# VachaLab/gorder

Measured on AMD Instinct MI355X. Metric: trajectory frames/sec, higher is better.
Workload: dtype f32

## Files before the change

### gorder_amd/csrc/trajectory_driver.h

```cpp
#pragma once

#include <atomic>
#include <chrono>
#include <condition_variable>
#include <deque>
#include <mutex>
#include <thread>

#include "../../include/gorder_xtc.h"

namespace {

struct TrajSlot {
    float *h_xyz = nullptr, *h_box = nullptr, *h_time = nullptr;
    float *d_xyz = nullptr, *d_box = nullptr;
    uint8_t *h_blob = nullptr, *d_blob = nullptr;
    gorder_xtc_frame_t *h_frames = nullptr, *d_frames = nullptr;
    float *d_box_in = nullptr;
    uint32_t *d_stat = nullptr, *d_short = nullptr, *h_stat = nullptr, *h_short = nullptr;
    XtcCheckpoint *d_cp = nullptr;
    std::vector<int64_t> file_pos;
    std::vector<uint32_t> file_idx;
    uint32_t prefix_q16 = 65536;
    uint32_t kinds = 0;
// ... 279 lines not shown
            {
                std::lock_guard<std::mutex> lk(pipe.mu);
                if (pipe.stop) return;
            }
            const auto t0 = std::chrono::steady_clock::now();
            const hipError_t e = alloc_slot(pipe.slot[k]);
            std::lock_guard<std::mutex> lk(pipe.mu);
            pipe.setup_s += seconds_since(t0);
            if (e != hipSuccess) { pipe.alloc_failed = true; return; }
            pipe.free_q.push_back(k);
            pipe.cv.notify_all();
        }
    });
    const double setup_s = seconds_since(t_start);

    gorder_xtc_pool *pool = nullptr;
    if (dev && gorder_xtc_pool_create(n_threads, &pool) != GORDER_XTC_OK) pool = nullptr;
    const char *forced_prefix = getenv("GORDER_HIP_PREFIX_Q16");
    const bool adapt_prefix = dev && has_xtc && !forced_prefix && !env_flag("GORDER_HIP_NO_PREFIX") && n_stop < n_file_atoms;
    if (dev && forced_prefix) pipe.prefix_q16.store((uint32_t)std::max(1l, std::min(65536l, atol(forced_prefix))));
    const bool verify = dev && has_xtc && (adapt_prefix || forced_prefix);
    const int device = h->device;
    std::thread reader([&, device]() {
        (void)hipSetDevice(device);
        uint64_t state = 0, analysed = shard_lo;
        double last_time = -INFINITY;
        uint32_t f = 0;
        gorder_xtc_reader *r = nullptr;
        bool done = shard_n == 0;
        uint32_t n_filled = 0;
        uint64_t to_skip = shard_lo, left = shard_n;
        auto give_up = [&](int st, const std::string &msg) {
            std::lock_guard<std::mutex> lk(pipe.mu);
            pipe.reader_status = st;
            pipe.reader_msg = msg;
            done = true;
        };
        while (!done) {
            int k = -1;
            {
                const auto t0 = std::chrono::steady_clock::now();
                std::unique_lock<std::mutex> lk(pipe.mu);
                pipe.cv.wait(lk, [&] { return pipe.stop || !pipe.free_q.empty(); });
                pipe.reader_stalled_s += seconds_since(t0);
                if (pipe.stop) break;
                k = pipe.free_q.front();
                pipe.free_q.pop_front();
            }
            TrajSlot &s = pipe.slot[k];
            const auto t_wait = std::chrono::steady_clock::now();
            if (s.copy_issued) (void)hipEventSynchronize(s.staged);
            const auto t1 = std::chrono::steady_clock::now();
            {
                std::lock_guard<std::mutex> lk(pipe.mu);
                pipe.reader_stalled_s += std::chrono::duration<double>(t1 - t_wait).count();
            }
            s.n = 0;
            s.blob_bytes = 0;
            uint32_t fill = batch;
            if (adapt_prefix && tr->batch_frames == 0 && f < tr->n_paths && file_is_xtc[f]) {
                if (n_filled == 0) fill = std::min(batch, 256u);
                else if (n_filled == 1) fill = std::min(batch, 1024u);
                else if (n_filled == 2) {
                    std::unique_lock<std::mutex> lk(pipe.mu);
                    pipe.cv.wait(lk, [&] { return pipe.stop || pipe.reports > 0; });
                }
            }
            s.prefix_q16 = pipe.prefix_q16.load();
            while (!done && s.n < fill) {
                if (left == 0) { done = true; break; }
                if (!r) {
                    if (f == tr->n_paths) { done = true; break; }
                    int st = gorder_xtc_open(tr->paths[f], tr->group, tr->n_group, &r);
                    if (st == GORDER_XTC_OK && gorder_xtc_n_atoms_out(r) != n_atoms) st = GORDER_XTC_ERR_ARGUMENT;
                    if (st != GORDER_XTC_OK) {
                        give_up(st, std::string("cannot read ") + tr->paths[f] +
                                        (st == GORDER_XTC_ERR_ARGUMENT ? ": atoms per frame differ from the tables" : ""));
                        break;
                    }
                }
                if (to_skip) {
                    const int64_t sk = gorder_xtc_skip_window(r, tr->begin_ps, tr->end_ps, tr->step, &state, &last_time, to_skip);
                    if (sk < 0) { give_up((int)sk, std::string("read error in ") + tr->paths[f]); break; }
                    to_skip -= (uint64_t)sk;
                    if (to_skip) {
                        gorder_xtc_close(r);
                        r = nullptr;
                        f++;
                        continue;
                    }
                }
                const uint64_t want = std::min<uint64_t>(fill - s.n, left);
                uint64_t used = 0;
                const int64_t got =
                    dev ? gorder_xtc_pack_window_ex(r, tr->begin_ps, tr->end_ps, tr->step, &state, &last_time,
                                                    s.h_blob + s.blob_bytes, blob_cap - s.blob_bytes, &used, s.h_frames + s.n,
                                                    s.h_box + 9u * (size_t)s.n, s.h_time + s.n, want, n_threads, pool,
                                                    s.prefix_q16, s.file_pos.data() + s.n)
                        : gorder_xtc_read_window_mt(r, tr->begin_ps, tr->end_ps, tr->step, &state, &last_time,
                                                    s.h_xyz + (size_t)s.n * n_atoms * 3u, s.h_box + 9u * (size_t)s.n,
                                                    s.h_time + s.n, want, n_threads);
                if (dev && got == GORDER_XTC_ERR_NO_SPACE) {
                    if (s.n > 0) break;
                    give_up(GORDER_XTC_ERR_ARGUMENT, std::string("a single frame of ") + tr->paths[f] + " does not fit the staging blob");
                    break;
                }
                if (got < 0) {
                    give_up((int)got, std::string("read error in ") + tr->paths[f]);
                    break;
                }
                if (got == 0) {
                    gorder_xtc_close(r);
                    r = nullptr;
                    f++;
                    continue;
                }
                if (dev) {
                    for (int64_t q = 0; q < got; q++) {
                        s.h_frames[s.n + (size_t)q].offset += s.blob_bytes;
                        s.file_idx[s.n + (size_t)q] = f;
                    }
                    s.blob_bytes += used;
                }
                s.n += (uint32_t)got;
                left -= (uint64_t)got;
            }
            if (pool) {
                const int cst = gorder_xtc_pool_wait(pool);
                if (cst != GORDER_XTC_OK && !done) give_up(cst, "read error while copying the compressed blocks");
                else if (cst != GORDER_XTC_OK) { std::lock_guard<std::mutex> lk(pipe.mu); if (pipe.reader_status == GORDER_XTC_OK) { pipe.reader_status = cst; pipe.reader_msg = "read error while copying the compressed blocks"; } }
            }
            const double dt = seconds_since(t1);
            std::lock_guard<std::mutex> lk(pipe.mu);
            pipe.decode_s += dt;
            if (s.n == 0 || pipe.reader_status != GORDER_XTC_OK) {
                pipe.free_q.push_front(k);
                break;
            }
            if (dev && (xtc_table_kinds(s.h_frames, s.n) & kXtcTableXtc)) n_filled++;
            s.fidx.resize((size_t)s.n);
            for (uint32_t q = 0; q < s.n; q++) s.fidx[q] = tr->first_frame_index + (analysed + q) * tr->step;
            analysed += s.n;
            pipe.filled_q.push_back(k);
            pipe.cv.notify_all();
        }
        if (r) gorder_xtc_close(r);
        std::lock_guard<std::mutex> lk(pipe.mu);
        pipe.reader_done = true;
        pipe.cv.notify_all();
    });

    int status = GORDER_OK;
    uint64_t frames = 0, batches = 0, bytes = 0, frames_fixed = 0;
    double starved_s = 0.0;
    std::string hip_msg;
    uint32_t need_q16 = 0;
    auto stage_a = [&](int k) {
        TrajSlot &s = pipe.slot[k];
        const size_t nx = (size_t)s.n * n_atoms * 3u * sizeof(float), nb = (size_t)s.n * 9u * sizeof(float);
        hipError_t e = hipSuccess;
        const hipStream_t feed = dev ? s.stream : copy_stream;
        if (s.compute_issued && !dev) e = hipStreamWaitEvent(feed, s.computed, 0);
// ... 124 lines not shown
            go = stage_b(front);
            any = true;
        }
        if (go && !any && !decoding.empty()) {
            std::unique_lock<std::mutex> lk(pipe.mu);
            pipe.cv.wait_for(lk, std::chrono::microseconds(100), [&] { return !pipe.filled_q.empty(); });
        }
    }
    {
        std::lock_guard<std::mutex> lk(pipe.mu);
        pipe.stop = true;
        pipe.cv.notify_all();
    }
    reader.join();
    allocator.join();
    if (pool) gorder_xtc_pool_destroy(pool);
    (void)hipStreamSynchronize(copy_stream);
    for (int k = 0; k < TrajPipe::kSlots; k++)
        if (pipe.slot[k].stream) (void)hipStreamSynchronize(pipe.slot[k].stream);
    const int sync_status = gorder_hip_synchronize(h);
    if (status == GORDER_OK) status = sync_status;
    else if (!hip_msg.empty()) h->err_msg = hip_msg;
    if (status == GORDER_OK && pipe.reader_status != GORDER_XTC_OK) {
        status = pipe.reader_status == GORDER_XTC_ERR_FORMAT ? GORDER_ERR_TRAJECTORY_FORMAT : GORDER_ERR_INVALID_ARGUMENT;
        h->err_msg = pipe.reader_msg + " (reader status " + std::to_string(pipe.reader_status) + ")";
    }
    if (stats) {
        stats->n_frames = frames;
        stats->n_batches = batches;
        stats->bytes_h2d = bytes;
        stats->seconds_total = seconds_since(t_start);
// ... 17 lines not shown
```

### gorder_amd/csrc/xtc_reader.cpp

```cpp
#include <algorithm>
#include <climits>
#include <cmath>
#include <cstdint>
#include <cstdio>
#include <cstring>
#include <string>
#include <string>
#include <atomic>
#include <chrono>
#include <condition_variable>
#include <deque>
#include <functional>
#include <memory>
#include <mutex>
#include <thread>
#include <immintrin.h>
#include <sys/mman.h>
#include <sys/stat.h>
#include <unistd.h>
#include <vector>

#include "../../include/gorder_xtc.h"

namespace {

const int kMagicInts[] = {
    0,       0,       0,       0,       0,       0,       0,       0,       0,       8,        10,       12,
    16,      20,      25,      32,      40,      50,      64,      80,      101,     128,      161,      203,
    256,     322,     406,     512,     645,     812,     1024,    1290,    1625,    2048,     2580,     3250,
    4096,    5060,    6501,    8192,    10321,   13003,   16384,   20642,   26007,   32768,    41285,    52015,
    65536,   82570,   104031,  131072,  165140,  208063,  262144,  330280,  416127,  524287,   660561,   832255,
    1048576, 1321122, 1664510, 2097152, 2642245, 3329021, 4194304, 5284491, 6658042, 8388607,  10568983, 13316085,
// ... 119 lines not shown
    float f;
    memcpy(&f, &u, 4);
    return f;
}

double bed(const uint8_t *p) {
    uint64_t u = 0;
    for (int k = 0; k < 8; k++) u = (u << 8) | p[k];
    double d;
    memcpy(&d, &u, 8);
    return d;
}

}

struct FileMap {
    const uint8_t *base = nullptr;
    size_t size = 0;
    ~FileMap() { if (base) munmap(const_cast<uint8_t *>(base), size); }
};

struct gorder_xtc_reader {
    std::string path;
    FILE *fp = nullptr;
    bool trr = false;
    bool gro = false;
    uint32_t natoms = 0;
    std::vector<uint32_t> group;
    std::vector<int32_t> slot_of;
    uint32_t n_needed = 0;
    std::vector<uint8_t> buf;
    std::vector<int> ints;
    std::shared_ptr<struct FileMap> map;
    bool map_tried = false;
};

namespace {

bool read_exact(FILE *fp, void *dst, size_t n) { return fread(dst, 1, n, fp) == n; }

int decode_ints(gorder_xtc_reader *r, const int minint[3], const int maxint[3], int smallidx, const uint8_t *data,
                size_t nbytes) {
    const uint32_t natoms = r->natoms;
    r->ints.resize((size_t)natoms * 3);
    uint32_t sizeint[3];
    int bitsizeint[3] = {0, 0, 0};
    for (int k = 0; k < 3; k++) {
        const int64_t s = (int64_t)maxint[k] - (int64_t)minint[k] + 1;
        if (s <= 0 || s > 0xffffffffll) return GORDER_XTC_ERR_FORMAT;
// ... 654 lines not shown
                float t = 0.0f;
                st = gorder_xtc_next(mine, xyz + i * nout * 3, box9 + i * 9, nullptr, &t, nullptr);
                if (st == GORDER_XTC_OK && time_ps) time_ps[i] = t;
            }
            gorder_xtc_close(mine);
            status[w] = st;
        });
    for (auto &th : pool) th.join();
    for (int st : status)
        if (st != GORDER_XTC_OK) return st == GORDER_XTC_EOF ? GORDER_XTC_ERR_FORMAT : st;
    return (int64_t)n;
}

}

struct gorder_xtc_pool {
    std::vector<std::thread> workers;
    std::mutex mu;
    std::condition_variable cv_work, cv_idle;
    std::deque<std::function<int()>> jobs;
    size_t running = 0;
    int status = GORDER_XTC_OK;
    bool stop = false;
    void loop() {
        for (;;) {
            std::function<int()> job;
            {
                std::unique_lock<std::mutex> lk(mu);
                cv_work.wait(lk, [&] { return stop || !jobs.empty(); });
                if (jobs.empty()) return;
                job = std::move(jobs.front());
                jobs.pop_front();
                running++;
            }
            const int st = job();
            std::lock_guard<std::mutex> lk(mu);
            if (st != GORDER_XTC_OK && status == GORDER_XTC_OK) status = st;
            running--;
            if (jobs.empty() && running == 0) cv_idle.notify_all();
        }
    }
};

extern "C" {

int gorder_xtc_pool_create(uint32_t n_threads, gorder_xtc_pool **out) {
    if (!out) return GORDER_XTC_ERR_ARGUMENT;
    gorder_xtc_pool *p = new gorder_xtc_pool();
    for (uint32_t w = 0; w < std::max(1u, n_threads); w++) p->workers.emplace_back([p] { p->loop(); });
    *out = p;
    return GORDER_XTC_OK;
}
int gorder_xtc_pool_wait(gorder_xtc_pool *p) {
    if (!p) return GORDER_XTC_ERR_ARGUMENT;
    std::unique_lock<std::mutex> lk(p->mu);
    p->cv_idle.wait(lk, [&] { return p->jobs.empty() && p->running == 0; });
    const int st = p->status;
    p->status = GORDER_XTC_OK;
    return st;
}
void gorder_xtc_pool_destroy(gorder_xtc_pool *p) {
    if (!p) return;
    {
        std::lock_guard<std::mutex> lk(p->mu);
// ... 74 lines not shown
    for (; i + 128 <= n; i += 128) {
        const __m256i a = _mm256_loadu_si256((const __m256i *)(src + i)), b = _mm256_loadu_si256((const __m256i *)(src + i + 32));
        const __m256i c = _mm256_loadu_si256((const __m256i *)(src + i + 64)), d = _mm256_loadu_si256((const __m256i *)(src + i + 96));
        _mm256_stream_si256((__m256i *)(dst + i), a);
        _mm256_stream_si256((__m256i *)(dst + i + 32), b);
        _mm256_stream_si256((__m256i *)(dst + i + 64), c);
        _mm256_stream_si256((__m256i *)(dst + i + 96), d);
    }
    if (i < n) memcpy(dst + i, src + i, n - i);
    _mm_sfence();
}
bool have_avx2() {
    static const bool yes = __builtin_cpu_supports("avx2");
    return yes;
}
int pack_copy(int fd, const FileMap *map, const PackSrc *src, size_t i0, size_t i1, uint8_t *blob) {
    const bool stream = map && map->base && have_avx2() && !getenv("GORDER_XTC_PREAD");
    for (size_t i = i0; i < i1; i++) {
        uint8_t *dst = blob + src[i].dst;
        size_t done = 0;
        if (stream && ((uintptr_t)dst & 31u) == 0 && (size_t)src[i].pos + src[i].n <= map->size) {
            stream_copy_avx2(dst, map->base + src[i].pos, src[i].n);
            done = src[i].n;
        }
        while (done < src[i].n) {
            const ssize_t g = pread(fd, dst + done, src[i].n - done, src[i].pos + (off_t)done);
            if (g <= 0) return GORDER_XTC_ERR_FORMAT;
            done += (size_t)g;
        }
        const size_t end = (size_t)((((uint64_t)src[i].n + 63u) & ~63ull) + 64u);
        memset(dst + src[i].n, 0, end - src[i].n);
    }
    return GORDER_XTC_OK;
}

int64_t pack_window_impl(gorder_xtc_reader *r, float begin_ps, float end_ps, uint32_t step, uint64_t *state,
                         double *last_time, uint8_t *blob, uint64_t blob_capacity, uint64_t *blob_bytes,
                         gorder_xtc_frame_t *frames, float *box9, float *time_ps, uint64_t capacity,
                         uint32_t n_threads, gorder_xtc_pool *pool, uint32_t prefix_q16 = 65536u, int64_t *file_pos = nullptr) {
    if (!r || !r->fp || r->gro || !state || !last_time || !blob || !blob_bytes || !frames || !box9 || step == 0)
        return GORDER_XTC_ERR_ARGUMENT;
    *blob_bytes = 0;
    const auto t_scan0 = std::chrono::steady_clock::now();
    std::vector<PackSrc> src;
    uint64_t used = 0;
    const uint32_t natoms = r->natoms;
    const int fd = fileno(r->fp);
    off_t pos = (off_t)ftello(r->fp);
    bool to_end = false;
    const uint64_t state_at_entry = *state;
    const double last_time_at_entry = *last_time;
    struct stat sb;
    const off_t file_end = fstat(fd, &sb) == 0 && S_ISREG(sb.st_mode) ? sb.st_size : (off_t)-1;
    if (!r->map_tried) {
        r->map_tried = true;
        if (file_end > 0) {
            void *m = mmap(nullptr, (size_t)file_end, PROT_READ, MAP_SHARED, fd, 0);
            if (m != MAP_FAILED) {
                (void)madvise(m, (size_t)file_end, MADV_SEQUENTIAL);
                r->map = std::make_shared<FileMap>();
                r->map->base = static_cast<const uint8_t *>(m);
                r->map->size = (size_t)file_end;
            }
        }
    }
    if (r->map && (getenv("GORDER_XTC_PREAD") || (file_end >= 0 && (size_t)file_end < r->map->size))) r->map.reset();
    const FileMap *map = r->map.get();
    auto fetch = [&](off_t at, uint8_t *dst, size_t n) -> ssize_t {
        if (map && map->base && at >= 0 && (size_t)at + n <= map->size) {
            memcpy(dst, map->base + at, n);
            return (ssize_t)n;
        }
        return pread(fd, dst, n, at);
    };
    const uint32_t n_stop = gorder_xtc_n_atoms_needed(r);
    while (src.size() < capacity) {
        const off_t pos0 = pos;
        uint8_t head[56 + 36];
        float t;
        float trr_box[9] = {0.0f, 0.0f, 0.0f, 0.0f, 0.0f, 0.0f, 0.0f, 0.0f, 0.0f};
        gorder_xtc_frame_t fr{};
        uint32_t block = 0;
        uint32_t copy = 0;
        off_t pos_block;
// ... 86 lines not shown
        }
        const size_t i = src.size();
        fr.offset = used;
        used += need;
        frames[i] = fr;
        for (int q = 0; q < 9; q++) box9[9 * i + q] = r->trr ? trr_box[q] : bef(head + 16 + 4 * q);
        if (time_ps) time_ps[i] = t;
        if (file_pos) file_pos[i] = (int64_t)pos0;
        src.push_back({pos_block, copy, fr.offset});
    }
    if (to_end ? fseek(r->fp, 0, SEEK_END) != 0 : fseeko(r->fp, pos, SEEK_SET) != 0) return GORDER_XTC_ERR_FORMAT;
    const size_t n = src.size();
    if (n == 0) return 0;
    const auto t_copy0 = std::chrono::steady_clock::now();
    if (pool) {
        const size_t nj = std::min<size_t>(pool->workers.size(), n);
        auto shared = std::make_shared<std::vector<PackSrc>>(std::move(src));
        const int fd2 = dup(fd);
        if (fd2 < 0) return GORDER_XTC_ERR_OPEN;
        auto left = std::make_shared<std::atomic<size_t>>(nj);
        std::shared_ptr<FileMap> keep = r->map;
        {
            std::lock_guard<std::mutex> lk(pool->mu);
            for (size_t w = 0; w < nj; w++) {
                const size_t i0 = n * w / nj, i1 = n * (w + 1) / nj;
                pool->jobs.emplace_back([shared, fd2, left, i0, i1, blob, keep]() {
                    const int st = pack_copy(fd2, keep.get(), shared->data(), i0, i1, blob);
                    if (left->fetch_sub(1) == 1) close(fd2);
                    return st;
                });
            }
        }
        pool->cv_work.notify_all();
        *blob_bytes = used;
        return (int64_t)n;
    }
    const uint32_t nt = (uint32_t)std::min<size_t>(std::max(1u, n_threads), n);
    std::vector<int> status(nt, GORDER_XTC_OK);
    auto work = [&](uint32_t w) { status[w] = pack_copy(fd, map, src.data(), n * w / nt, n * (w + 1) / nt, blob); };
    if (nt == 1) {
        work(0);
    } else {
        std::vector<std::thread> threads;
        for (uint32_t w = 0; w < nt; w++) threads.emplace_back(work, w);
        for (auto &th : threads) th.join();
    }
    for (int st : status)
        if (st != GORDER_XTC_OK) return st;
    if (getenv("GORDER_XTC_PACK_TIMING")) {
        const auto t1 = std::chrono::steady_clock::now();
        fprintf(stderr, "pack_window: %zu frames, scan %.3f ms, copy %.3f ms (%u threads, %.1f MB)\n", n,
                std::chrono::duration<double, std::milli>(t_copy0 - t_scan0).count(),
                std::chrono::duration<double, std::milli>(t1 - t_copy0).count(), nt, used / 1e6);
    }
// ... 24 lines not shown
    if (!r || !r->fp || !xyz) return GORDER_XTC_ERR_ARGUMENT;
    if (fseeko(r->fp, (off_t)file_pos, SEEK_SET) != 0) return GORDER_XTC_ERR_FORMAT;
    return gorder_xtc_next(r, xyz, box9, nullptr, nullptr, nullptr);
}

int64_t gorder_xtc_pack_window_pool(gorder_xtc_reader *r, float begin_ps, float end_ps, uint32_t step, uint64_t *state,
                                    double *last_time, uint8_t *blob, uint64_t blob_capacity, uint64_t *blob_bytes,
                                    gorder_xtc_frame_t *frames, float *box9, float *time_ps, uint64_t capacity,
                                    gorder_xtc_pool *pool) {
    if (!pool) return GORDER_XTC_ERR_ARGUMENT;
    return pack_window_impl(r, begin_ps, end_ps, step, state, last_time, blob, blob_capacity, blob_bytes, frames, box9,
                            time_ps, capacity, 1, pool);
}

}
```

### gorder_amd/xtc.py

```python
from __future__ import annotations

import ctypes as C
from typing import Optional, Sequence

import numpy as np

from .abi import load_library

_bound = False


def _lib():
    global _bound
    lib = load_library()
    if not _bound:
        vp = C.c_void_p
        lib.gorder_xtc_open.argtypes = [C.c_char_p, vp, C.c_uint32, C.POINTER(vp)]
        lib.gorder_xtc_close.argtypes = [vp]
        lib.gorder_xtc_close.restype = None
        lib.gorder_xtc_n_atoms_file.argtypes = [vp]
        lib.gorder_xtc_n_atoms_file.restype = C.c_uint32
        lib.gorder_xtc_n_atoms_out.argtypes = [vp]
        lib.gorder_xtc_n_atoms_out.restype = C.c_uint32
        lib.gorder_xtc_next.argtypes = [vp, vp, vp, C.POINTER(C.c_int64), C.POINTER(C.c_float), C.POINTER(C.c_float)]
# ... 223 lines not shown
    state, last = C.c_uint64(0), C.c_double(float("-inf"))
    total = 0
    for path in paths:
        r = C.c_void_p()
        st = lib.gorder_xtc_open(path.encode(), None, 0, C.byref(r))
        if st != 0:
            raise IOError(f"cannot open {path}: status {st}")
        try:
            n = lib.gorder_xtc_skip_window(r, begin, end, step, C.byref(state), C.byref(last), 2 ** 64 - 1)
            if n < 0:
                raise IOError(f"{path}: XTC read error {n}")
            total += n
        finally:
            lib.gorder_xtc_close(r)
    return total
```

### include/gorder_xtc.h

```cpp
#ifndef GORDER_XTC_H
#define GORDER_XTC_H

#include <stddef.h>
#include <stdint.h>

#ifdef __cplusplus
extern "C" {
#endif

typedef struct gorder_xtc_reader gorder_xtc_reader;

typedef enum {
    GORDER_XTC_OK = 0,
    GORDER_XTC_EOF = 1,
    GORDER_XTC_ERR_OPEN = -1,
    GORDER_XTC_ERR_FORMAT = -2,
    GORDER_XTC_ERR_ARGUMENT = -3,
    GORDER_XTC_ERR_NO_SPACE = -4
} gorder_xtc_status_t;

int gorder_xtc_open(const char *path, const uint32_t *group, uint32_t n_group, gorder_xtc_reader **out);
void gorder_xtc_close(gorder_xtc_reader *r);
uint32_t gorder_xtc_n_atoms_file(const gorder_xtc_reader *r);
uint32_t gorder_xtc_n_atoms_out(const gorder_xtc_reader *r);
// ... 32 lines not shown
typedef struct gorder_xtc_pool gorder_xtc_pool;
int gorder_xtc_pool_create(uint32_t n_threads, gorder_xtc_pool **out);
int gorder_xtc_pool_wait(gorder_xtc_pool *pool);
void gorder_xtc_pool_destroy(gorder_xtc_pool *pool);
int64_t gorder_xtc_pack_window_pool(gorder_xtc_reader *r, float begin_ps, float end_ps, uint32_t step, uint64_t *state,
                                    double *last_time, uint8_t *blob, uint64_t blob_capacity, uint64_t *blob_bytes,
                                    gorder_xtc_frame_t *frames, float *box9, float *time_ps, uint64_t capacity,
                                    gorder_xtc_pool *pool);

int64_t gorder_xtc_pack_window_ex(gorder_xtc_reader *r, float begin_ps, float end_ps, uint32_t step, uint64_t *state,
                                  double *last_time, uint8_t *blob, uint64_t blob_capacity, uint64_t *blob_bytes,
                                  gorder_xtc_frame_t *frames, float *box9, float *time_ps, uint64_t capacity,
                                  uint32_t n_threads, gorder_xtc_pool *pool, uint32_t prefix_q16, int64_t *file_pos);
int gorder_xtc_read_at(gorder_xtc_reader *r, int64_t file_pos, float *xyz, float *box9);

int gorder_xtc_probe(const char *path, uint32_t *n_atoms, uint64_t *file_bytes, uint32_t *first_frame_bytes);
enum { GORDER_XTC_FORMAT_OTHER = 0, GORDER_XTC_FORMAT_XTC = 1, GORDER_XTC_FORMAT_TRR = 2 };
int gorder_xtc_probe_format(const char *path, int *format, uint32_t *n_atoms, uint64_t *file_bytes,
                            uint32_t *first_frame_bytes);
int gorder_xtc_is_xtc(const gorder_xtc_reader *r);
int gorder_xtc_can_pack(const gorder_xtc_reader *r);
uint32_t gorder_xtc_n_atoms_needed(const gorder_xtc_reader *r);

typedef struct gorder_xtc_writer gorder_xtc_writer;
int gorder_xtc_writer_open(const char *path, uint32_t n_atoms, float precision, gorder_xtc_writer **out);
int gorder_xtc_writer_add(gorder_xtc_writer *w, const float *xyz, const float *box9, int64_t step, float time_ps);
void gorder_xtc_writer_close(gorder_xtc_writer *w);

#ifdef __cplusplus
}
// ... 3 lines not shown
```

Measured before the change: 21.07 million.

## Add trajectory feeder with ticketed async block copies and background unmap reaper

Replaces the reader thread's inline open/skip/pack loop with a new feeder object. The feeder hands out tickets for the pooled compressed-block copies, so the reader can start filling the next slot before publishing the previous one, keeping one batch in flight. File unmapping (madvise DONTNEED plus munmap) moves to a background reaper thread, taking page-release cost off the critical path. Staging-event waits now run only when the event is still pending. This adds more threads and ordering complexity, which could cause races or extra contention.

Measured after the change: 20.40 million. 3.2% lower.

```diff
diff --git a/gorder_amd/csrc/trajectory_driver.h b/gorder_amd/csrc/trajectory_driver.h
--- a/gorder_amd/csrc/trajectory_driver.h
+++ b/gorder_amd/csrc/trajectory_driver.h
@@ -317,8 +317,7 @@
     });
     const double setup_s = seconds_since(t_start);
 
-    gorder_xtc_pool *pool = nullptr;
-    if (dev && gorder_xtc_pool_create(n_threads, &pool) != GORDER_XTC_OK) pool = nullptr;
+    const bool feed_timing = getenv("GORDER_XTC_PACK_TIMING") != nullptr;
     const char *forced_prefix = getenv("GORDER_HIP_PREFIX_Q16");
     const bool adapt_prefix = dev && has_xtc && !forced_prefix && !env_flag("GORDER_HIP_NO_PREFIX") && n_stop < n_file_atoms;
     if (dev && forced_prefix) pipe.prefix_q16.store((uint32_t)std::max(1l, std::min(65536l, atol(forced_prefix))));
@@ -326,129 +325,150 @@
     const int device = h->device;
     std::thread reader([&, device]() {
         (void)hipSetDevice(device);
-        uint64_t state = 0, analysed = shard_lo;
-        double last_time = -INFINITY;
-        uint32_t f = 0;
-        gorder_xtc_reader *r = nullptr;
+        const auto t_reader = std::chrono::steady_clock::now();
+        double stalled = 0.0;
+        uint64_t analysed = shard_lo;
         bool done = shard_n == 0;
         uint32_t n_filled = 0;
-        uint64_t to_skip = shard_lo, left = shard_n;
+        gorder_xtc_feed *feed = nullptr;
+        {
+            gorder_xtc_feed_config_t fc{};
+            fc.paths = tr->paths;
+            fc.n_paths = tr->n_paths;
+            fc.group = tr->group;
+            fc.n_group = tr->n_group;
+            fc.begin_ps = tr->begin_ps;
+            fc.end_ps = tr->end_ps;
+            fc.step = tr->step;
+            fc.n_atoms_out = n_atoms;
+            fc.skip_frames = shard_lo;
+            fc.max_frames = shard_n;
+            fc.n_threads = n_threads;
+            fc.flags = feed_timing ? GORDER_XTC_FEED_TIMING : 0u;
+            if (!done && gorder_xtc_feed_open(&fc, &feed) != GORDER_XTC_OK) feed = nullptr;
+        }
         auto give_up = [&](int st, const std::string &msg) {
             std::lock_guard<std::mutex> lk(pipe.mu);
-            pipe.reader_status = st;
-            pipe.reader_msg = msg;
+            if (pipe.reader_status == GORDER_XTC_OK) {
+                pipe.reader_status = st;
+                pipe.reader_msg = msg;
+            }
             done = true;
         };
+        if (!done && !feed) give_up(GORDER_XTC_ERR_ARGUMENT, "cannot start the trajectory feeder");
+        struct Pending { int k; uint64_t ticket; };
+        std::deque<Pending> pending;
+        bool copy_failed = false;
+        auto publish_oldest = [&]() {
+            const Pending p = pending.front();
+            pending.pop_front();
+            TrajSlot &s = pipe.slot[p.k];
+            const int cst = gorder_xtc_feed_wait(feed, p.ticket);
+            if (cst != GORDER_XTC_OK && !copy_failed) {
+                give_up(cst, "read error while copying the compressed blocks");
+                copy_failed = true;
+            }
+            std::lock_guard<std::mutex> lk(pipe.mu);
+            if (copy_failed) {
+                pipe.free_q.push_front(p.k);
+                return;
+            }
+            s.fidx.resize((size_t)s.n);
+            for (uint32_t q = 0; q < s.n; q++) s.fidx[q] = tr->first_frame_index + (analysed + q) * tr->step;
+            analysed += s.n;
+            pipe.filled_q.push_back(p.k);
+            pipe.cv.notify_all();
+        };
+        auto publish_all = [&]() { while (!pending.empty()) publish_oldest(); };
         while (!done) {
             int k = -1;
             {
+                std::unique_lock<std::mutex> lk(pipe.mu);
+                if (pipe.stop) break;
+                if (!pipe.free_q.empty()) {
+                    k = pipe.free_q.front();
+                    pipe.free_q.pop_front();
+                }
+            }
+            if (k < 0) {
+                publish_all();
                 const auto t0 = std::chrono::steady_clock::now();
                 std::unique_lock<std::mutex> lk(pipe.mu);
                 pipe.cv.wait(lk, [&] { return pipe.stop || !pipe.free_q.empty(); });
-                pipe.reader_stalled_s += seconds_since(t0);
+                stalled += seconds_since(t0);
                 if (pipe.stop) break;
                 k = pipe.free_q.front();
                 pipe.free_q.pop_front();
             }
             TrajSlot &s = pipe.slot[k];
-            const auto t_wait = std::chrono::steady_clock::now();
-            if (s.copy_issued) (void)hipEventSynchronize(s.staged);
-            const auto t1 = std::chrono::steady_clock::now();
-            {
-                std::lock_guard<std::mutex> lk(pipe.mu);
-                pipe.reader_stalled_s += std::chrono::duration<double>(t1 - t_wait).count();
+            if (s.copy_issued && hipEventQuery(s.staged) != hipSuccess) {
+                publish_all();
+                const auto t_wait = std::chrono::steady_clock::now();
+                (void)hipEventSynchronize(s.staged);
+                stalled += seconds_since(t_wait);
             }
             s.n = 0;
             s.blob_bytes = 0;
             uint32_t fill = batch;
+            const uint32_t f = gorder_xtc_feed_next_file(feed);
             if (adapt_prefix && tr->batch_frames == 0 && f < tr->n_paths && file_is_xtc[f]) {
                 if (n_filled == 0) fill = std::min(batch, 256u);
                 else if (n_filled == 1) fill = std::min(batch, 1024u);
                 else if (n_filled == 2) {
+                    publish_all();
                     std::unique_lock<std::mutex> lk(pipe.mu);
                     pipe.cv.wait(lk, [&] { return pipe.stop || pipe.reports > 0; });
                 }
             }
             s.prefix_q16 = pipe.prefix_q16.load();
-            while (!done && s.n < fill) {
-                if (left == 0) { done = true; break; }
-                if (!r) {
-                    if (f == tr->n_paths) { done = true; break; }
-                    int st = gorder_xtc_open(tr->paths[f], tr->group, tr->n_group, &r);
-                    if (st == GORDER_XTC_OK && gorder_xtc_n_atoms_out(r) != n_atoms) st = GORDER_XTC_ERR_ARGUMENT;
-                    if (st != GORDER_XTC_OK) {
-                        give_up(st, std::string("cannot read ") + tr->paths[f] +
-                                        (st == GORDER_XTC_ERR_ARGUMENT ? ": atoms per frame differ from the tables" : ""));
-                        break;
-                    }
-                }
-                if (to_skip) {
-                    const int64_t sk = gorder_xtc_skip_window(r, tr->begin_ps, tr->end_ps, tr->step, &state, &last_time, to_skip);
-                    if (sk < 0) { give_up((int)sk, std::string("read error in ") + tr->paths[f]); break; }
-                    to_skip -= (uint64_t)sk;
-                    if (to_skip) {
-                        gorder_xtc_close(r);
-                        r = nullptr;
-                        f++;
-                        continue;
-                    }
-                }
-                const uint64_t want = std::min<uint64_t>(fill - s.n, left);
-                uint64_t used = 0;
-                const int64_t got =
-                    dev ? gorder_xtc_pack_window_ex(r, tr->begin_ps, tr->end_ps, tr->step, &state, &last_time,
-                                                    s.h_blob + s.blob_bytes, blob_cap - s.blob_bytes, &used, s.h_frames + s.n,
-                                                    s.h_box + 9u * (size_t)s.n, s.h_time + s.n, want, n_threads, pool,
-                                                    s.prefix_q16, s.file_pos.data() + s.n)
-                        : gorder_xtc_read_window_mt(r, tr->begin_ps, tr->end_ps, tr->step, &state, &last_time,
-                                                    s.h_xyz + (size_t)s.n * n_atoms * 3u, s.h_box + 9u * (size_t)s.n,
-                                                    s.h_time + s.n, want, n_threads);
-                if (dev && got == GORDER_XTC_ERR_NO_SPACE) {
-                    if (s.n > 0) break;
-                    give_up(GORDER_XTC_ERR_ARGUMENT, std::string("a single frame of ") + tr->paths[f] + " does not fit the staging blob");
-                    break;
-                }
-                if (got < 0) {
-                    give_up((int)got, std::string("read error in ") + tr->paths[f]);
-                    break;
-                }
-                if (got == 0) {
-                    gorder_xtc_close(r);
-                    r = nullptr;
-                    f++;
-                    continue;
-                }
-                if (dev) {
-                    for (int64_t q = 0; q < got; q++) {
-                        s.h_frames[s.n + (size_t)q].offset += s.blob_bytes;
-                        s.file_idx[s.n + (size_t)q] = f;
-                    }
-                    s.blob_bytes += used;
-                }
-                s.n += (uint32_t)got;
-                left -= (uint64_t)got;
-            }
-            if (pool) {
-                const int cst = gorder_xtc_pool_wait(pool);
-                if (cst != GORDER_XTC_OK && !done) give_up(cst, "read error while copying the compressed blocks");
-                else if (cst != GORDER_XTC_OK) { std::lock_guard<std::mutex> lk(pipe.mu); if (pipe.reader_status == GORDER_XTC_OK) { pipe.reader_status = cst; pipe.reader_msg = "read error while copying the compressed blocks"; } }
-            }
-            const double dt = seconds_since(t1);
-            std::lock_guard<std::mutex> lk(pipe.mu);
-            pipe.decode_s += dt;
-            if (s.n == 0 || pipe.reader_status != GORDER_XTC_OK) {
+            gorder_xtc_feed_slot_t fs{};
+            if (dev) {
+                fs.blob = s.h_blob;
+                fs.blob_capacity = blob_cap;
+                fs.frames = s.h_frames;
+                fs.file_pos = s.file_pos.data();
+                fs.file_idx = s.file_idx.data();
+            } else {
+                fs.xyz = s.h_xyz;
+            }
+            fs.box9 = s.h_box;
+            fs.time_ps = s.h_time;
+            fs.capacity = batch;
+            uint64_t ticket = 0;
+            const int64_t got = gorder_xtc_feed_fill(feed, &fs, fill, s.prefix_q16, &s.blob_bytes, &ticket);
+            if (got < 0) {
+                publish_all();
+                give_up((int)got, gorder_xtc_feed_message(feed));
+            }
+            if (got <= 0) {
+                done = true;
+                std::lock_guard<std::mutex> lk(pipe.mu);
                 pipe.free_q.push_front(k);
                 break;
             }
+            s.n = (uint32_t)got;
             if (dev && (xtc_table_kinds(s.h_frames, s.n) & kXtcTableXtc)) n_filled++;
-            s.fidx.resize((size_t)s.n);
-            for (uint32_t q = 0; q < s.n; q++) s.fidx[q] = tr->first_frame_index + (analysed + q) * tr->step;
-            analysed += s.n;
-            pipe.filled_q.push_back(k);
-            pipe.cv.notify_all();
-        }
-        if (r) gorder_xtc_close(r);
+            pending.push_back({k, ticket});
+            if (!dev || pending.size() > 1) publish_oldest();
+        }
+        publish_all();
+        if (feed) {
+            if (feed_timing) {
+                gorder_xtc_feed_stats_t fst;
+                gorder_xtc_feed_get_stats(feed, &fst);
+                double busy = 0.0;
+                uint64_t faults = 0;
+                for (uint32_t w = 0; w < std::min(64u, fst.n_workers); w++) { busy += fst.worker_busy_s[w]; faults += fst.worker_minflt[w]; }
+                fprintf(stderr, "trajectory feeder: scan %.3f s, open %.3f s, close %.3f s, waiting for copies %.3f s, waiting for a slot %.3f s; "
+                                "%u workers busy %.3f s in %llu jobs (%.2f GB, %llu minor faults); release %.3f s\n",
+                        fst.scan_s, fst.open_s, fst.close_s, fst.wait_s, stalled, fst.n_workers, busy, (unsigned long long)fst.jobs,
+                        fst.bytes_copied / 1e9, (unsigned long long)faults, fst.reaper_s);
+            }
+            gorder_xtc_feed_close(feed);
+        }
         std::lock_guard<std::mutex> lk(pipe.mu);
+        pipe.decode_s = std::max(0.0, seconds_since(t_reader) - stalled);
+        pipe.reader_stalled_s += stalled;
         pipe.reader_done = true;
         pipe.cv.notify_all();
     });
@@ -603,7 +623,6 @@
     }
     reader.join();
     allocator.join();
-    if (pool) gorder_xtc_pool_destroy(pool);
     (void)hipStreamSynchronize(copy_stream);
     for (int k = 0; k < TrajPipe::kSlots; k++)
         if (pipe.slot[k].stream) (void)hipStreamSynchronize(pipe.slot[k].stream);
diff --git a/gorder_amd/csrc/xtc_reader.cpp b/gorder_amd/csrc/xtc_reader.cpp
--- a/gorder_amd/csrc/xtc_reader.cpp
+++ b/gorder_amd/csrc/xtc_reader.cpp
@@ -16,6 +16,7 @@
 #include <thread>
 #include <immintrin.h>
 #include <sys/mman.h>
+#include <sys/resource.h>
 #include <sys/stat.h>
 #include <unistd.h>
 #include <vector>
@@ -165,11 +166,76 @@
 
 }
 
+struct MapReaper;
 struct FileMap {
     const uint8_t *base = nullptr;
     size_t size = 0;
-    ~FileMap() { if (base) munmap(const_cast<uint8_t *>(base), size); }
+    std::shared_ptr<MapReaper> reaper;
+    ~FileMap();
 };
+
+struct MapReaper {
+    struct Range { const uint8_t *base; size_t size; };
+    std::thread th;
+    std::mutex mu;
+    std::condition_variable cv, cv_idle;
+    std::deque<Range> release;
+    bool stop = false, busy = false, keep_pages = false;
+    double busy_s = 0.0;
+    uint64_t minflt = 0;
+    static constexpr size_t kPiece = (size_t)8 << 20;
+    void start() { th = std::thread([this] { loop(); }); }
+    void give(const uint8_t *base, size_t size) {
+        {
+            std::lock_guard<std::mutex> lk(mu);
+            release.push_back({base, size});
+        }
+        cv.notify_one();
+    }
+    void flush() {
+        std::unique_lock<std::mutex> lk(mu);
+        cv_idle.wait(lk, [&] { return release.empty() && !busy; });
+    }
+    void finish() {
+        {
+            std::lock_guard<std::mutex> lk(mu);
+            stop = true;
+        }
+        cv.notify_one();
+        if (th.joinable()) th.join();
+    }
+    void loop() {
+        for (;;) {
+            Range rg{nullptr, 0};
+            {
+                std::unique_lock<std::mutex> lk(mu);
+                busy = false;
+                if (release.empty()) cv_idle.notify_all();
+                cv.wait(lk, [&] { return stop || !release.empty(); });
+                if (release.empty()) return;
+                rg = release.front();
+                release.pop_front();
+                busy = true;
+            }
+            const auto t0 = std::chrono::steady_clock::now();
+            uint8_t *b = const_cast<uint8_t *>(rg.base);
+            if (!keep_pages)
+                for (size_t off = 0; off < rg.size; off += kPiece) (void)madvise(b + off, std::min(kPiece, rg.size - off), MADV_DONTNEED);
+            munmap(b, rg.size);
+            struct rusage ru;
+            const bool have_ru = getrusage(RUSAGE_THREAD, &ru) == 0;
+            std::lock_guard<std::mutex> lk(mu);
+            busy_s += std::chrono::duration<double>(std::chrono::steady_clock::now() - t0).count();
+            if (have_ru) minflt = (uint64_t)ru.ru_minflt;
+        }
+    }
+};
+
+FileMap::~FileMap() {
+    if (!base) return;
+    if (reaper) reaper->give(base, size);
+    else munmap(const_cast<uint8_t *>(base), size);
+}
 
 struct gorder_xtc_reader {
     std::string path;
@@ -184,6 +250,7 @@
     std::vector<int> ints;
     std::shared_ptr<struct FileMap> map;
     bool map_tried = false;
+    std::shared_ptr<struct MapReaper> reaper;
 };
 
 namespace {
@@ -868,17 +935,29 @@
 
 }
 
+struct CopyGroup {
+    size_t pending = 0;
+    int status = GORDER_XTC_OK;
+};
 struct gorder_xtc_pool {
+    struct Job {
+        std::function<int()> fn;
+        std::shared_ptr<CopyGroup> group;
+    };
     std::vector<std::thread> workers;
     std::mutex mu;
     std::condition_variable cv_work, cv_idle;
-    std::deque<std::function<int()>> jobs;
+    std::deque<Job> jobs;
     size_t running = 0;
     int status = GORDER_XTC_OK;
     bool stop = false;
-    void loop() {
+    bool timing = false;
+    std::vector<double> busy_s;
+    std::vector<uint64_t> minflt;
+    uint64_t n_jobs = 0;
+    void loop(size_t w) {
         for (;;) {
-            std::function<int()> job;
+            Job job;
             {
                 std::unique_lock<std::mutex> lk(mu);
                 cv_work.wait(lk, [&] { return stop || !jobs.empty(); });
@@ -887,21 +966,49 @@
                 jobs.pop_front();
                 running++;
             }
-            const int st = job();
+            const auto t0 = std::chrono::steady_clock::now();
+            const int st = job.fn();
+            job.fn = nullptr;
+            double dt = 0.0;
+            struct rusage ru;
+            bool have_ru = false;
+            if (timing) {
+                dt = std::chrono::duration<double>(std::chrono::steady_clock::now() - t0).count();
+                have_ru = getrusage(RUSAGE_THREAD, &ru) == 0;
+            }
             std::lock_guard<std::mutex> lk(mu);
-            if (st != GORDER_XTC_OK && status == GORDER_XTC_OK) status = st;
+            busy_s[w] += dt;
+            if (have_ru) minflt[w] = (uint64_t)ru.ru_minflt;
+            n_jobs++;
             running--;
+            if (job.group) {
+                if (st != GORDER_XTC_OK && job.group->status == GORDER_XTC_OK) job.group->status = st;
+                if (--job.group->pending == 0) cv_idle.notify_all();
+            } else if (st != GORDER_XTC_OK && status == GORDER_XTC_OK) {
+                status = st;
+            }
             if (jobs.empty() && running == 0) cv_idle.notify_all();
         }
     }
 };
+
+namespace {
+int pool_wait_group(gorder_xtc_pool *p, CopyGroup *g) {
+    std::unique_lock<std::mutex> lk(p->mu);
+    p->cv_idle.wait(lk, [&] { return g->pending == 0; });
+    return g->status;
+}
+}
 
 extern "C" {
 
 int gorder_xtc_pool_create(uint32_t n_threads, gorder_xtc_pool **out) {
     if (!out) return GORDER_XTC_ERR_ARGUMENT;
     gorder_xtc_pool *p = new gorder_xtc_pool();
-    for (uint32_t w = 0; w < std::max(1u, n_threads); w++) p->workers.emplace_back([p] { p->loop(); });
+    const uint32_t nw = std::max(1u, n_threads);
+    p->busy_s.assign(nw, 0.0);
+    p->minflt.assign(nw, 0);
+    for (uint32_t w = 0; w < nw; w++) p->workers.emplace_back([p, w] { p->loop(w); });
     *out = p;
     return GORDER_XTC_OK;
 }
@@ -1006,8 +1113,8 @@
     static const bool yes = __builtin_cpu_supports("avx2");
     return yes;
 }
-int pack_copy(int fd, const FileMap *map, const PackSrc *src, size_t i0, size_t i1, uint8_t *blob) {
-    const bool stream = map && map->base && have_avx2() && !getenv("GORDER_XTC_PREAD");
+int pack_copy(int fd, const FileMap *map, const PackSrc *src, size_t i0, size_t i1, uint8_t *blob, bool use_pread) {
+    const bool stream = map && map->base && have_avx2() && !use_pread;
     for (size_t i = i0; i < i1; i++) {
         uint8_t *dst = blob + src[i].dst;
         size_t done = 0;
@@ -1026,10 +1133,18 @@
     return GORDER_XTC_OK;
 }
 
+struct FeedJobs {
+    std::shared_ptr<CopyGroup> group;
+    uint64_t job_bytes = 0;
+    bool scan_pread = false;
+    uint64_t *bytes_copied = nullptr;
+};
+
 int64_t pack_window_impl(gorder_xtc_reader *r, float begin_ps, float end_ps, uint32_t step, uint64_t *state,
                          double *last_time, uint8_t *blob, uint64_t blob_capacity, uint64_t *blob_bytes,
                          gorder_xtc_frame_t *frames, float *box9, float *time_ps, uint64_t capacity,
-                         uint32_t n_threads, gorder_xtc_pool *pool, uint32_t prefix_q16 = 65536u, int64_t *file_pos = nullptr) {
+                         uint32_t n_threads, gorder_xtc_pool *pool, uint32_t prefix_q16 = 65536u, int64_t *file_pos = nullptr,
+                         const FeedJobs *feed = nullptr) {
     if (!r || !r->fp || r->gro || !state || !last_time || !blob || !blob_bytes || !frames || !box9 || step == 0)
         return GORDER_XTC_ERR_ARGUMENT;
     *blob_bytes = 0;
@@ -1053,13 +1168,16 @@
                 r->map = std::make_shared<FileMap>();
                 r->map->base = static_cast<const uint8_t *>(m);
                 r->map->size = (size_t)file_end;
-            }
-        }
-    }
-    if (r->map && (getenv("GORDER_XTC_PREAD") || (file_end >= 0 && (size_t)file_end < r->map->size))) r->map.reset();
+                r->map->reaper = r->reaper;
+            }
+        }
+    }
+    const bool use_pread = getenv("GORDER_XTC_PREAD") != nullptr;
+    if (r->map && (use_pread || (file_end >= 0 && (size_t)file_end < r->map->size))) r->map.reset();
     const FileMap *map = r->map.get();
+    const bool scan_pread = feed && feed->scan_pread;
     auto fetch = [&](off_t at, uint8_t *dst, size_t n) -> ssize_t {
-        if (map && map->base && at >= 0 && (size_t)at + n <= map->size) {
+        if (!scan_pread && map && map->base && at >= 0 && (size_t)at + n <= map->size) {
             memcpy(dst, map->base + at, n);
             return (ssize_t)n;
         }
@@ -1176,21 +1294,40 @@
     if (n == 0) return 0;
     const auto t_copy0 = std::chrono::steady_clock::now();
     if (pool) {
-        const size_t nj = std::min<size_t>(pool->workers.size(), n);
+        std::vector<size_t> cut(1, 0);
+        if (feed && feed->job_bytes) {
+            uint64_t acc = 0;
+            for (size_t i = 0; i < n; i++) {
+                if (acc && acc + src[i].n > feed->job_bytes) {
+                    cut.push_back(i);
+                    acc = 0;
+                }
+                acc += src[i].n;
+            }
+            cut.push_back(n);
+        } else {
+            const size_t shares = std::min<size_t>(pool->workers.size(), n);
+            for (size_t w = 0; w < shares; w++) cut.push_back(n * (w + 1) / shares);
+        }
+        const size_t nj = cut.size() - 1;
+        if (feed && feed->bytes_copied)
+            for (size_t i = 0; i < n; i++) *feed->bytes_copied += src[i].n;
         auto shared = std::make_shared<std::vector<PackSrc>>(std::move(src));
         const int fd2 = dup(fd);
         if (fd2 < 0) return GORDER_XTC_ERR_OPEN;
         auto left = std::make_shared<std::atomic<size_t>>(nj);
         std::shared_ptr<FileMap> keep = r->map;
+        std::shared_ptr<CopyGroup> group = feed ? feed->group : nullptr;
         {
             std::lock_guard<std::mutex> lk(pool->mu);
+            if (group) group->pending += nj;
             for (size_t w = 0; w < nj; w++) {
-                const size_t i0 = n * w / nj, i1 = n * (w + 1) / nj;
-                pool->jobs.emplace_back([shared, fd2, left, i0, i1, blob, keep]() {
-                    const int st = pack_copy(fd2, keep.get(), shared->data(), i0, i1, blob);
+                const size_t i0 = cut[w], i1 = cut[w + 1];
+                pool->jobs.push_back({[shared, fd2, left, i0, i1, blob, keep, use_pread]() {
+                    const int st = pack_copy(fd2, keep.get(), shared->data(), i0, i1, blob, use_pread);
                     if (left->fetch_sub(1) == 1) close(fd2);
                     return st;
-                });
+                }, group});
             }
         }
         pool->cv_work.notify_all();
@@ -1199,7 +1336,7 @@
     }
     const uint32_t nt = (uint32_t)std::min<size_t>(std::max(1u, n_threads), n);
     std::vector<int> status(nt, GORDER_XTC_OK);
-    auto work = [&](uint32_t w) { status[w] = pack_copy(fd, map, src.data(), n * w / nt, n * (w + 1) / nt, blob); };
+    auto work = [&](uint32_t w) { status[w] = pack_copy(fd, map, src.data(), n * w / nt, n * (w + 1) / nt, blob, use_pread); };
     if (nt == 1) {
         work(0);
     } else {
@@ -1254,3 +1391,208 @@
 }
 
 }
+
+constexpr uint64_t kFeedJobBytes = (uint64_t)1 << 20;
+
+struct gorder_xtc_feed {
+    std::vector<std::string> paths;
+    std::vector<uint32_t> group;
+    float begin_ps = 0.0f, end_ps = -1.0f;
+    uint32_t step = 1, n_atoms_out = 0, n_threads = 1, flags = 0;
+    uint64_t job_bytes = kFeedJobBytes;
+    gorder_xtc_pool *pool = nullptr;
+    std::shared_ptr<MapReaper> reaper;
+    gorder_xtc_reader *r = nullptr;
+    uint32_t fi = 0;
+    uint64_t state = 0, to_skip = 0, left = 0;
+    double last_time = -INFINITY;
+    int failed = GORDER_XTC_OK;
+    std::string msg;
+    std::mutex mu;
+    std::vector<std::pair<uint64_t, std::shared_ptr<CopyGroup>>> groups;
+    uint64_t next_ticket = 1;
+    double scan_s = 0.0, open_s = 0.0, close_s = 0.0, wait_s = 0.0;
+    uint64_t bytes_copied = 0;
+    void close_file() {
+        const auto t0 = std::chrono::steady_clock::now();
+        gorder_xtc_close(r);
+        r = nullptr;
+        close_s += std::chrono::duration<double>(std::chrono::steady_clock::now() - t0).count();
+    }
+    int64_t fail(int st, const std::string &what) {
+        failed = st;
+        msg = what;
+        return st;
+    }
+};
+
+extern "C" {
+
+int gorder_xtc_feed_open(const gorder_xtc_feed_config_t *cfg, gorder_xtc_feed **out) {
+    if (!cfg || !out || (!cfg->paths && cfg->n_paths) || cfg->step == 0) return GORDER_XTC_ERR_ARGUMENT;
+    *out = nullptr;
+    gorder_xtc_feed *f = new gorder_xtc_feed();
+    for (uint32_t k = 0; k < cfg->n_paths; k++) f->paths.emplace_back(cfg->paths[k] ? cfg->paths[k] : "");
+    if (cfg->group && cfg->n_group) f->group.assign(cfg->group, cfg->group + cfg->n_group);
+    f->begin_ps = cfg->begin_ps;
+    f->end_ps = cfg->end_ps;
+    f->step = cfg->step;
+    f->n_atoms_out = cfg->n_atoms_out;
+    f->n_threads = std::max(1u, cfg->n_threads);
+    f->flags = cfg->flags;
+    f->to_skip = cfg->skip_frames;
+    f->left = cfg->max_frames;
+    if (cfg->job_bytes) f->job_bytes = cfg->job_bytes;
+    if (const char *e = getenv("GORDER_XTC_FEED_JOB_BYTES"))
+        if (atoll(e) > 0) f->job_bytes = (uint64_t)atoll(e);
+    if (gorder_xtc_pool_create(f->n_threads, &f->pool) != GORDER_XTC_OK) {
+        delete f;
+        return GORDER_XTC_ERR_ARGUMENT;
+    }
+    f->pool->timing = (cfg->flags & GORDER_XTC_FEED_TIMING) != 0;
+    f->reaper = std::make_shared<MapReaper>();
+    f->reaper->keep_pages = (cfg->flags & GORDER_XTC_FEED_KEEP_PAGES) != 0;
+    f->reaper->start();
+    *out = f;
+    return GORDER_XTC_OK;
+}
+
+int64_t gorder_xtc_feed_fill(gorder_xtc_feed *f, const gorder_xtc_feed_slot_t *slot, uint64_t max_frames, uint32_t prefix_q16,
+                             uint64_t *blob_bytes, uint64_t *ticket) {
+    if (!f || !slot || !blob_bytes || !ticket || !slot->box9 || (!slot->xyz && (!slot->blob || !slot->frames)))
+        return GORDER_XTC_ERR_ARGUMENT;
+    *blob_bytes = 0;
+    *ticket = 0;
+    if (f->failed != GORDER_XTC_OK) return f->failed;
+    const bool pack = slot->xyz == nullptr;
+    const uint64_t fill = std::min(max_frames, slot->capacity);
+    FeedJobs jobs;
+    jobs.group = std::make_shared<CopyGroup>();
+    jobs.job_bytes = f->job_bytes;
+    jobs.scan_pread = (f->flags & GORDER_XTC_FEED_SCAN_MAPPED) == 0;
+    jobs.bytes_copied = &f->bytes_copied;
+    uint64_t n = 0, bytes = 0;
+    while (n < fill && f->left > 0) {
+        if (!f->r) {
+            if (f->fi == f->paths.size()) break;
+            const std::string &path = f->paths[f->fi];
+            const auto t0 = std::chrono::steady_clock::now();
+            int st = gorder_xtc_open(path.c_str(), f->group.empty() ? nullptr : f->group.data(), (uint32_t)f->group.size(), &f->r);
+            f->open_s += std::chrono::duration<double>(std::chrono::steady_clock::now() - t0).count();
+            if (st == GORDER_XTC_OK && f->n_atoms_out && gorder_xtc_n_atoms_out(f->r) != f->n_atoms_out) st = GORDER_XTC_ERR_ARGUMENT;
+            if (st != GORDER_XTC_OK)
+                return f->fail(st, "cannot read " + path + (st == GORDER_XTC_ERR_ARGUMENT ? ": atoms per frame differ from the tables" : ""));
+            f->r->reaper = f->reaper;
+        }
+        const std::string &path = f->paths[f->fi];
+        const auto t0 = std::chrono::steady_clock::now();
+        if (f->to_skip) {
+            const int64_t sk = gorder_xtc_skip_window(f->r, f->begin_ps, f->end_ps, f->step, &f->state, &f->last_time, f->to_skip);
+            f->scan_s += std::chrono::duration<double>(std::chrono::steady_clock::now() - t0).count();
+            if (sk < 0) return f->fail((int)sk, "read error in " + path);
+            f->to_skip -= (uint64_t)sk;
+            if (f->to_skip) {
+                f->close_file();
+                f->fi++;
+            }
+            continue;
+        }
+        const uint64_t want = std::min(fill - n, f->left);
+        uint64_t used = 0;
+        const int64_t got =
+            pack ? pack_window_impl(f->r, f->begin_ps, f->end_ps, f->step, &f->state, &f->last_time, slot->blob + bytes,
+                                    slot->blob_capacity - bytes, &used, slot->frames + n, slot->box9 + 9u * n,
+                                    slot->time_ps ? slot->time_ps + n : nullptr, want, f->n_threads, f->pool,
+                                    prefix_q16 ? prefix_q16 : 65536u, slot->file_pos ? slot->file_pos + n : nullptr, &jobs)
+                 : gorder_xtc_read_window_mt(f->r, f->begin_ps, f->end_ps, f->step, &f->state, &f->last_time,
+                                             slot->xyz + n * (uint64_t)gorder_xtc_n_atoms_out(f->r) * 3u, slot->box9 + 9u * n,
+                                             slot->time_ps ? slot->time_ps + n : nullptr, want, f->n_threads);
+        f->scan_s += std::chrono::duration<double>(std::chrono::steady_clock::now() - t0).count();
+        if (pack && got == GORDER_XTC_ERR_NO_SPACE) {
+            if (n > 0) break;
+            return f->fail(GORDER_XTC_ERR_ARGUMENT, "a single frame of " + path + " does not fit the staging blob");
+        }
+        if (got < 0) return f->fail((int)got, "read error in " + path);
+        if (got == 0) {
+            f->close_file();
+            f->fi++;
+            continue;
+        }
+        if (pack) {
+            for (int64_t q = 0; q < got; q++) {
+                slot->frames[n + (uint64_t)q].offset += bytes;
+                if (slot->file_idx) slot->file_idx[n + (uint64_t)q] = f->fi;
+            }
+            bytes += used;
+        }
+        n += (uint64_t)got;
+        f->left -= (uint64_t)got;
+    }
+    *blob_bytes = bytes;
+    std::lock_guard<std::mutex> lk(f->mu);
+    *ticket = f->next_ticket++;
+    f->groups.emplace_back(*ticket, jobs.group);
+    return (int64_t)n;
+}
+
+int gorder_xtc_feed_wait(gorder_xtc_feed *f, uint64_t ticket) {
+    if (!f) return GORDER_XTC_ERR_ARGUMENT;
+    std::shared_ptr<CopyGroup> g;
+    {
+        std::lock_guard<std::mutex> lk(f->mu);
+        for (size_t k = 0; k < f->groups.size(); k++)
+            if (f->groups[k].first == ticket) {
+                g = f->groups[k].second;
+                f->groups.erase(f->groups.begin() + (ptrdiff_t)k);
+                break;
+            }
+    }
+    if (!g) return GORDER_XTC_ERR_ARGUMENT;
+    const auto t0 = std::chrono::steady_clock::now();
+    const int st = pool_wait_group(f->pool, g.get());
+    const double dt = std::chrono::duration<double>(std::chrono::steady_clock::now() - t0).count();
+    std::lock_guard<std::mutex> lk(f->mu);
+    f->wait_s += dt;
+    return st;
+}
+
+const char *gorder_xtc_feed_message(const gorder_xtc_feed *f) { return f ? f->msg.c_str() : ""; }
+uint32_t gorder_xtc_feed_next_file(const gorder_xtc_feed *f) { return f ? f->fi : 0; }
+
+void gorder_xtc_feed_get_stats(gorder_xtc_feed *f, gorder_xtc_feed_stats_t *out) {
+    if (!f || !out) return;
+    memset(out, 0, sizeof(*out));
+    (void)gorder_xtc_pool_wait(f->pool);
+    f->reaper->flush();
+    {
+        std::lock_guard<std::mutex> lk(f->mu);
+        out->scan_s = f->scan_s;
+        out->open_s = f->open_s;
+        out->close_s = f->close_s;
+        out->wait_s = f->wait_s;
+        out->bytes_copied = f->bytes_copied;
+    }
+    {
+        std::lock_guard<std::mutex> lk(f->pool->mu);
+        out->jobs = f->pool->n_jobs;
+        out->n_workers = (uint32_t)f->pool->workers.size();
+        for (size_t w = 0; w < std::min<size_t>(64, f->pool->workers.size()); w++) {
+            out->worker_busy_s[w] = f->pool->busy_s[w];
+            out->worker_minflt[w] = f->pool->minflt[w];
+        }
+    }
+    std::lock_guard<std::mutex> lk(f->reaper->mu);
+    out->reaper_s = f->reaper->busy_s;
+    out->reaper_minflt = f->reaper->minflt;
+}
+
+void gorder_xtc_feed_close(gorder_xtc_feed *f) {
+    if (!f) return;
+    (void)gorder_xtc_pool_wait(f->pool);
+    if (f->r) gorder_xtc_close(f->r);
+    gorder_xtc_pool_destroy(f->pool);
+    f->reaper->finish();
+    delete f;
+}
+
+}
diff --git a/gorder_amd/xtc.py b/gorder_amd/xtc.py
--- a/gorder_amd/xtc.py
+++ b/gorder_amd/xtc.py
@@ -261,3 +261,103 @@
         finally:
             lib.gorder_xtc_close(r)
     return total
+
+
+FEED_KEEP_PAGES, FEED_SCAN_MAPPED, FEED_TIMING = 1, 2, 4
+
+
+class CFeedConfig(C.Structure):
+    _fields_ = [("paths", C.POINTER(C.c_char_p)), ("n_paths", C.c_uint32), ("group", C.c_void_p), ("n_group", C.c_uint32),
+                ("begin_ps", C.c_float), ("end_ps", C.c_float), ("step", C.c_uint32), ("n_atoms_out", C.c_uint32),
+                ("skip_frames", C.c_uint64), ("max_frames", C.c_uint64), ("n_threads", C.c_uint32), ("flags", C.c_uint32),
+                ("job_bytes", C.c_uint64)]
+
+
+class CFeedSlot(C.Structure):
+    _fields_ = [("blob", C.c_void_p), ("blob_capacity", C.c_uint64), ("frames", C.c_void_p), ("file_pos", C.c_void_p),
+                ("file_idx", C.c_void_p), ("xyz", C.c_void_p), ("box9", C.c_void_p), ("time_ps", C.c_void_p),
+                ("capacity", C.c_uint64)]
+
+
+class CFeedStats(C.Structure):
+    _fields_ = [("scan_s", C.c_double), ("open_s", C.c_double), ("close_s", C.c_double), ("wait_s", C.c_double),
+                ("reaper_s", C.c_double), ("reaper_minflt", C.c_uint64), ("bytes_copied", C.c_uint64), ("jobs", C.c_uint64),
+                ("n_workers", C.c_uint32), ("worker_busy_s", C.c_double * 64), ("worker_minflt", C.c_uint64 * 64)]
+
+
+class FeedError(IOError):
+
+    def __init__(self, status, message, slot, slots):
+        super().__init__(f"slot {slot}: status {status}: {message}")
+        self.status, self.message, self.slot, self.slots = status, message, slot, slots
+
+
+def feed_slots(paths: Sequence[str], capacity: int, blob_capacity: int, group: Optional[np.ndarray] = None,
+               begin: float = 0.0, end: float = -1.0, step: int = 1, fills: Optional[Sequence[int]] = None,
+               in_flight: int = 1, threads: int = 2, job_bytes: int = 0, prefix_q16: int = 65536, skip: int = 0,
+               max_frames: int = 2 ** 64 - 1, flags: int = 0, n_atoms_out: int = 0):
+    from .abi import CXtcFrame
+    lib = _lib()
+    vp = C.c_void_p
+    lib.gorder_xtc_feed_open.argtypes = [C.POINTER(CFeedConfig), C.POINTER(vp)]
+    lib.gorder_xtc_feed_fill.argtypes = [vp, C.POINTER(CFeedSlot), C.c_uint64, C.c_uint32, C.POINTER(C.c_uint64),
+                                         C.POINTER(C.c_uint64)]
+    lib.gorder_xtc_feed_fill.restype = C.c_int64
+    lib.gorder_xtc_feed_wait.argtypes = [vp, C.c_uint64]
+    lib.gorder_xtc_feed_message.argtypes = [vp]
+    lib.gorder_xtc_feed_message.restype = C.c_char_p
+    lib.gorder_xtc_feed_get_stats.argtypes = [vp, C.POINTER(CFeedStats)]
+    lib.gorder_xtc_feed_get_stats.restype = None
+    lib.gorder_xtc_feed_close.argtypes = [vp]
+    lib.gorder_xtc_feed_close.restype = None
+    grp = None if group is None else np.ascontiguousarray(group, dtype=np.uint32)
+    cpaths = (C.c_char_p * len(paths))(*[p.encode() for p in paths])
+    cfg = CFeedConfig(cpaths, len(paths), None if grp is None else grp.ctypes.data, 0 if grp is None else grp.size, begin, end,
+                      step, n_atoms_out, skip, max_frames, threads, flags, job_bytes)
+    feed = vp()
+    st = lib.gorder_xtc_feed_open(C.byref(cfg), C.byref(feed))
+    if st != 0:
+        raise IOError(f"cannot open the feeder: status {st}")
+    n_buf = in_flight + 1
+    bufs = [{"blob": np.empty(blob_capacity, np.uint8), "frames": (CXtcFrame * capacity)(), "box": np.empty((capacity, 3, 3), np.float32),
+             "time": np.empty(capacity, np.float32), "file_idx": np.zeros(capacity, np.uint32),
+             "file_pos": np.zeros(capacity, np.int64)} for _ in range(n_buf)]
+    done, queued = [], []
+
+    def finish_oldest():
+        k, ticket, n, used = queued.pop(0)
+        st = lib.gorder_xtc_feed_wait(feed, ticket)
+        if st != 0:
+            raise FeedError(st, "read error while copying the compressed blocks", len(done), done)
+        b = bufs[k % n_buf]
+        done.append({"n": n, "blob": b["blob"][:used].copy(), "frames": np.frombuffer(b["frames"], dtype=np.dtype(CXtcFrame))[:n].copy(),
+                     "box": b["box"][:n].copy(), "time": b["time"][:n].copy(), "file_idx": b["file_idx"][:n].copy(),
+                     "file_pos": b["file_pos"][:n].copy()})
+
+    try:
+        k = 0
+        while True:
+            if len(queued) == in_flight:
+                finish_oldest()
+            b = bufs[k % n_buf]
+            b["blob"][:] = 0xA5
+            slot = CFeedSlot(b["blob"].ctypes.data, blob_capacity, C.cast(b["frames"], vp), b["file_pos"].ctypes.data,
+                             b["file_idx"].ctypes.data, None, b["box"].ctypes.data, b["time"].ctypes.data, capacity)
+            used, ticket = C.c_uint64(0), C.c_uint64(0)
+            want = capacity if fills is None or k >= len(fills) else fills[k]
+            got = lib.gorder_xtc_feed_fill(feed, C.byref(slot), want, prefix_q16, C.byref(used), C.byref(ticket))
+            if got < 0:
+                while queued:
+                    finish_oldest()
+                raise FeedError(got, lib.gorder_xtc_feed_message(feed).decode(), len(done), done)
+            if got == 0:
+                break
+            queued.append((k, ticket.value, got, used.value))
+            k += 1
+        while queued:
+            finish_oldest()
+        stats = CFeedStats()
+        lib.gorder_xtc_feed_get_stats(feed, C.byref(stats))
+        return done, {"jobs": stats.jobs, "bytes_copied": stats.bytes_copied}
+    finally:
+        lib.gorder_xtc_feed_close(feed)
diff --git a/include/gorder_xtc.h b/include/gorder_xtc.h
--- a/include/gorder_xtc.h
+++ b/include/gorder_xtc.h
@@ -70,6 +70,54 @@
                                   uint32_t n_threads, gorder_xtc_pool *pool, uint32_t prefix_q16, int64_t *file_pos);
 int gorder_xtc_read_at(gorder_xtc_reader *r, int64_t file_pos, float *xyz, float *box9);
 
+typedef struct gorder_xtc_feed gorder_xtc_feed;
+enum {
+    GORDER_XTC_FEED_KEEP_PAGES = 1u,
+    GORDER_XTC_FEED_SCAN_MAPPED = 2u,
+    GORDER_XTC_FEED_TIMING = 4u
+};
+typedef struct {
+    const char *const *paths;
+    uint32_t n_paths;
+    const uint32_t *group;
+    uint32_t n_group;
+    float begin_ps, end_ps;
+    uint32_t step;
+    uint32_t n_atoms_out;
+    uint64_t skip_frames;
+    uint64_t max_frames;
+    uint32_t n_threads;
+    uint32_t flags;
+    uint64_t job_bytes;
+} gorder_xtc_feed_config_t;
+typedef struct {
+    uint8_t *blob;
+    uint64_t blob_capacity;
+    gorder_xtc_frame_t *frames;
+    int64_t *file_pos;
+    uint32_t *file_idx;
+    float *xyz;
+    float *box9, *time_ps;
+    uint64_t capacity;
+} gorder_xtc_feed_slot_t;
+typedef struct {
+    double scan_s, open_s, close_s, wait_s;
+    double reaper_s;
+    uint64_t reaper_minflt, bytes_copied, jobs;
+    uint32_t n_workers;
+    double worker_busy_s[64];
+    uint64_t worker_minflt[64];
+} gorder_xtc_feed_stats_t;
+
+int gorder_xtc_feed_open(const gorder_xtc_feed_config_t *cfg, gorder_xtc_feed **out);
+int64_t gorder_xtc_feed_fill(gorder_xtc_feed *f, const gorder_xtc_feed_slot_t *slot, uint64_t max_frames, uint32_t prefix_q16,
+                             uint64_t *blob_bytes, uint64_t *ticket);
+int gorder_xtc_feed_wait(gorder_xtc_feed *f, uint64_t ticket);
+const char *gorder_xtc_feed_message(const gorder_xtc_feed *f);
+uint32_t gorder_xtc_feed_next_file(const gorder_xtc_feed *f);
+void gorder_xtc_feed_get_stats(gorder_xtc_feed *f, gorder_xtc_feed_stats_t *out);
+void gorder_xtc_feed_close(gorder_xtc_feed *f);
+
 int gorder_xtc_probe(const char *path, uint32_t *n_atoms, uint64_t *file_bytes, uint32_t *first_frame_bytes);
 enum { GORDER_XTC_FORMAT_OTHER = 0, GORDER_XTC_FORMAT_XTC = 1, GORDER_XTC_FORMAT_TRR = 2 };
 int gorder_xtc_probe_format(const char *path, int *format, uint32_t *n_atoms, uint64_t *file_bytes,
```
